# micropilot/myosuite-mjx

Hardware: AMD Instinct MI355X
Metric: env-steps/s (whole node) myoHandPoseRandom-v0 batch 4096 (higher is better)
Workload: dtype f32

## Files before the change

__graft_entry__.py:

```python
import os
import subprocess
import sys

ROOT = os.path.dirname(os.path.abspath(__file__))
sys.path.insert(0, ROOT)


def build() -> None:
    from myosuite_mjx_amd import capi
    capi.build_library(force=True, verbose=True)
    capi.build_diagnostic("poison", verbose=True)
    subprocess.check_call(["make", "-C", os.path.join(ROOT, "oracle"), "-s"])
    if os.path.isdir("/root/reference/myosuite") and os.environ.get("MYO_RECOMPILE_MODELS") == "1":
        subprocess.check_call([sys.executable, os.path.join(ROOT, "tools", "compile_models.py")])
    import myosuite_mjx_amd
    import ctypes
    lib = ctypes.CDLL(capi.LIB_PATH)
    for sym in ("myo_model_load", "myo_batch_create", "myo_step", "myo_obs", "myo_reset"):
        getattr(lib, sym)
    print("build ok:", capi.LIB_PATH)


def smoke() -> None:
    import numpy as np
    from myosuite_mjx_amd import capi, model as M
    from oracle.oracle import Oracle
# ... 32 lines not shown
```

include/myo_hip.h:

```cpp
#ifndef MYO_HIP_H
#define MYO_HIP_H
#include <stddef.h>
#include <stdint.h>
#ifdef __cplusplus
extern "C" {
#endif

typedef struct myo_model myo_model;
typedef struct myo_batch myo_batch;

enum { MYO_OK = 0, MYO_E_ARG = -1, MYO_E_BLOB = -2, MYO_E_HIP = -3, MYO_E_UNSUPPORTED = -4, MYO_E_NOMEM = -5 };

typedef struct myo_dims {
  int nq, nv, nu, na, nbody, ntendon, nsite, nlink, obs_dim, env_lds_bytes, lanes_per_env, ncon_max;
  float timestep;
} myo_dims;

typedef enum myo_field {
  MYO_F_QPOS = 0,
  MYO_F_QVEL,
  MYO_F_ACT,
  MYO_F_CTRL,
  MYO_F_WARMSTART,
  MYO_F_TIME,
// ... 19 lines not shown
  MYO_F_BODYMASS_RANGE,
  MYO_F_COUNT
} myo_field;

enum {
  MYO_F_BODYPOS = MYO_F_COUNT,
  MYO_F_BODYPOS_RANGE,
};

enum { MYO_FLAG_BAD_STATE = 1, MYO_FLAG_BAD_QACC = 2, MYO_FLAG_CONTACT_OVERFLOW = 4, MYO_FLAG_CAND_OVERFLOW = 8,
       MYO_FLAG_SCHED_TIMEOUT = 16  };

enum {
  MYO_F_BODYQUAT = MYO_F_BODYPOS_RANGE + 1,
  MYO_F_BODYQUAT_RANGE,
};

enum {
  MYO_ACTMAP_NONE = 0,
  MYO_ACTMAP_MUSCLE_SIGMOID = 1,
  MYO_ACTMAP_SIGMOID_FATIGUE = 2,
  MYO_ACTMAP_SIGMOID_REAFFERENTATION = 3,
  MYO_ACTMAP_CTRLRANGE = 4
};

typedef enum myo_task { MYO_TASK_NONE = 0, MYO_TASK_POSE = 1, MYO_TASK_REACH = 2, MYO_TASK_WALK = 3,
                        MYO_TASK_STAND = 5,
                        MYO_TASK_TRACK = 6,
                        MYO_TASK_KEYTURN = 7,
                        MYO_TASK_PEN = 8,
// ... 120 lines not shown
```

myosuite_mjx_amd/capi.py:

```python
from __future__ import annotations

import ctypes as C
import os
import subprocess

import numpy as np

_HERE = os.path.dirname(os.path.abspath(__file__))
LIB_PATH = os.environ.get("MYO_HIP_LIB") or os.path.join(_HERE, "libmyo_hip.so")
SRC_PATH = os.path.join(_HERE, "csrc", "myo_hip.hip")

(F_QPOS, F_QVEL, F_ACT, F_CTRL, F_WARMSTART, F_TIME, F_TARGET, F_OBS, F_REWARD, F_DONE, F_SOLVED, F_FLAGS, F_DIAG,
 F_QACC, F_TENLEN, F_ACTFORCE, F_SITEXPOS, F_ELAPSED, F_ACTION, F_FATIGUE, F_HFIELD, F_GEOMSIZE, F_LINKX, F_METRICS,
 F_BODYMASS, F_BODYMASS_RANGE, F_BODYPOS, F_BODYPOS_RANGE) = range(28)
F_BODYQUAT, F_BODYQUAT_RANGE = 28, 29
INT_FIELDS = (F_FLAGS, F_DIAG, F_ELAPSED)
BENCH_OBS, BENCH_FRESH_ACTIONS, BENCH_AUTORESET = 1, 2, 4
ACTMAP_NONE, ACTMAP_MUSCLE_SIGMOID, ACTMAP_SIGMOID_FATIGUE, ACTMAP_SIGMOID_REAFFERENTATION, ACTMAP_CTRLRANGE = 0, 1, 2, 3, 4
TASK_NONE, TASK_POSE, TASK_REACH = 0, 1, 2
TASK_HOLD = 4
TASK_STAND = 5
TASK_TRACK = 6
TASK_KEYTURN = 7
TASK_PEN = 8
TASK_BAODING = 9
TASK_DIE = 10
FLAG_BAD_STATE, FLAG_BAD_QACC, FLAG_CONTACT_OVERFLOW, FLAG_CAND_OVERFLOW = 1, 2, 4, 8


class Dims(C.Structure):
    _fields_ = [(n, C.c_int) for n in ("nq", "nv", "nu", "na", "nbody", "ntendon", "nsite", "nlink", "obs_dim",
# ... 50 lines not shown
def build_library(force=False, verbose=False):
    csrc = os.path.dirname(SRC_PATH)
    newest = max(os.path.getmtime(os.path.join(csrc, f)) for f in os.listdir(csrc) if f.endswith((".hip", ".h")))
    newest = max(newest, os.path.getmtime(os.path.join(os.path.dirname(os.path.dirname(csrc)), "include", "myo_hip.h")))
    if not force and os.path.exists(LIB_PATH) and os.path.getmtime(LIB_PATH) >= newest:
        return LIB_PATH
    hipcc = os.environ.get("HIPCC", "/opt/rocm/bin/hipcc")
    cmd = [hipcc, *HIPCC_FLAGS, "-shared", "-fPIC", "-o", LIB_PATH, SRC_PATH]
    if verbose:
        print(" ".join(cmd))
    subprocess.check_call(cmd)
    return LIB_PATH


def build_diagnostic(variant, force=False, verbose=False):
    flag = {"poison": "-DMYO_POISON=1", "stamps": "-DMYO_STAMPS=1"}[variant]
    out = os.path.join(os.path.dirname(LIB_PATH), f"libmyo_hip_{variant}.so")
    csrc = os.path.dirname(SRC_PATH)
    newest = max(os.path.getmtime(os.path.join(csrc, f)) for f in os.listdir(csrc) if f.endswith((".hip", ".h")))
    if not force and os.path.exists(out) and os.path.getmtime(out) >= newest:
        return out
    hipcc = os.environ.get("HIPCC", "/opt/rocm/bin/hipcc")
    cmd = [hipcc, *HIPCC_FLAGS, flag, "-shared", "-fPIC", "-o", out, SRC_PATH]
    if verbose:
        print(" ".join(cmd))
    subprocess.check_call(cmd)
    return out


_lib = None

# ... 314 lines not shown
```

myosuite_mjx_amd/csrc/myo_common.h:

```cpp
#ifndef MYO_COMMON_H
#define MYO_COMMON_H

#include <hip/hip_runtime.h>

#include <algorithm>
#include <utility>
#include <cmath>
#include <cstdint>
#include <cstdio>
#include <cstdlib>
#include <cstring>
#include <mutex>
#include <string>
#include <vector>

#include "../../include/myo_hip.h"

#define MINVALF 1e-15f
#define MAXVALF 1e10f
#define MINIMPF 0.0001f
#define MAXIMPF 0.9999f
#define NCON 32
#define NCAND 128
#ifndef LS_FLOOR
// ... 72 lines not shown
  float obj_p[3], obj_R[9], wrist_p[3];
  float lift_z, obj_err_scale, base_err_scale, lift_bonus_mag, qpos_w, qpos_err_scale, qvel_w, qvel_err_scale;
  float obj_fail2, base_fail2, qpos_fail;
  float w_pose, w_object, w_bonus, w_penalty;
  float* ref;
  int ref_pitch;
  float* metrics;
  uint64_t seed;
};

struct DevBatch {
  int B;
  float *qpos, *qvel, *act, *ctrl, *warm, *time, *target, *obs, *reward, *done, *solved, *qacc, *tenlen, *actforce, *sitexpos;
  int *flags, *diag, *elapsed, *episode;
  int* mprw;
  float* fatigue;
  float fat_dt;
  int reaf_epl, reaf_eip;
  float* hfield;
  float* gsize;
  int gsize_cg;
  float* bmass;
  float* bmass_range;
  float* linkc;
  int nbody;
  float* bpos;
  float* bpos_range;
  int bpos_link;
  float* ovf;
  int* ovf_cand;
// ... 163 lines not shown
```

myosuite_mjx_amd/csrc/myo_hip.hip:

```cpp
#include "myo_common.h"
#include "myo_physics.h"
#include "myo_task_track.h"
#include "myo_kernel_lanes.h"
#include "myo_kernel_wave.h"
#include "myo_kernels_aux.h"
#include "myo_host.h"
#include "myo_task_keyturn.h"
#include "myo_task_pen.h"
#include "myo_task_baoding.h"
#include "myo_task_die.h"
#include "myo_task_myodm.h"
#include "myo_host_model.h"

extern "C" {

const char* myo_last_error(void) { return g_err.c_str(); }
int myo_version(void) { return 1; }

int myo_model_load(const void* blobv, size_t nbytes, int device, myo_model** out) {
  if (!blobv || !out || nbytes < 16) return fail(MYO_E_ARG, "myo_model_load: bad arguments");
  const Blob B{(const uint8_t*)blobv};
  uint32_t ver;
  memcpy(&ver, B.p + 4, 4);
  if (memcmp(B.p, "MYOB", 4) || ver != 3) return fail(MYO_E_BLOB, "myo_model_load: not a MYOB v3 blob");
// ... 44 lines not shown
  DevBatch& d = b->db;
  d.B = B;
  int nv = m->dm.nv, nu = m->dm.nu, nq = m->nq, rc;
  b->ntarget_alloc = nv > 24 ? nv : 24;
  b->obs_alloc = 3 * nv + 4 * nu + 64;
#define BA(ptr, n) if ((rc = balloc(b, (void**)&ptr, (size_t)(n) * 4))) { myo_batch_free(b); return rc; }
  BA(d.qpos, (size_t)B * nq) BA(d.qvel, (size_t)B * nv) BA(d.act, (size_t)B * nu) BA(d.ctrl, (size_t)B * nu) BA(d.warm, (size_t)B * nv)
  BA(d.time, B) BA(d.target, (size_t)B * b->ntarget_alloc) BA(d.obs, (size_t)B * b->obs_alloc) BA(d.reward, B) BA(d.done, B)
  BA(d.solved, B) BA(d.qacc, (size_t)B * nv) BA(d.tenlen, (size_t)B * nu) BA(d.actforce, (size_t)B * nu) BA(d.sitexpos, (size_t)B * 24)
  BA(d.flags, B) BA(d.diag, (size_t)B * 8) BA(d.elapsed, B) BA(d.episode, B) BA(d.mprw, (size_t)B * 64)
  BA(b->d_tlo, b->ntarget_alloc) BA(b->d_thi, b->ntarget_alloc) BA(b->d_init, nq) BA(b->d_jlo, nv) BA(b->d_jhi, nv) BA(b->d_rnd, 4 * (size_t)nq)
  BA(b->d_action, (size_t)B * nu)
  BA(d.fatigue, (size_t)B * 3 * nu)
  d.hfield = nullptr; d.gsize = nullptr; d.gsize_cg = -1;
  d.ovf = nullptr; d.ovf_cand = nullptr; d.ovf_row = 0; d.ovf_rows = 0; d.linkx = nullptr; d.track = nullptr; d.env_offset = 0;
  if (m->trk) { BA(d.linkx, (size_t)B * 12 * m->dm.nl) }
  if (m->wave_ok) {
    const int kc = m->wave_cfg == 0 ? 8 : 20, nj = m->trk ? 4 : 3;
    d.ovf_row = 8 + nj * kc + (kc + 3) / 4 + (m->trk ? TRK_STATE : 0);
    d.ovf_rows = m->trk ? NCX2 : NCX;
    BA(d.ovf, (size_t)B * d.ovf_rows * d.ovf_row) BA(d.ovf_cand, (size_t)B * NCANDX)
  }
  if (m->dw.hf.on) { BA(d.hfield, (size_t)B * m->dw.hf.nrow * m->dw.hf.ncol) }
  BA(b->d_initv, nv) BA(b->d_init2, nq) BA(b->d_initv2, nv) BA(b->d_fatvec, nu)
  { void* pw = nullptr; if ((rc = balloc(b, &pw, sizeof(DevWalk)))) { myo_batch_free(b); return rc; } b->d_walk = (DevWalk*)pw; }
  BA(b->d_stamps, (size_t)B * 12 * 3 * 2)
  BA(b->d_order, B)
  b->sched_stride = (B + 7) / 8 + 1;
  BA(b->d_sched, 32 + B + 64)
#undef BA
// ... 316 lines not shown
    case MYO_F_ACT: *p = d.act; *pitch = *width = nu; break;
    case MYO_F_CTRL: *p = d.ctrl; *pitch = *width = nu; break;
    case MYO_F_WARMSTART: *p = d.warm; *pitch = *width = nv; break;
    case MYO_F_TIME: *p = d.time; *pitch = *width = 1; break;
    case MYO_F_TARGET: *p = d.target; *pitch = *width = b->task.ntarget > 0 ? b->task.ntarget : 1; break;
    case MYO_F_OBS: *p = d.obs; *pitch = *width = b->task.obs_dim > 0 ? b->task.obs_dim : 1; break;
    case MYO_F_REWARD: *p = d.reward; *pitch = *width = 1; break;
    case MYO_F_DONE: *p = d.done; *pitch = *width = 1; break;
    case MYO_F_SOLVED: *p = d.solved; *pitch = *width = 1; break;
    case MYO_F_FLAGS: *p = d.flags; *pitch = *width = 1; break;
    case MYO_F_DIAG: *p = d.diag; *pitch = *width = 8; break;
    case MYO_F_QACC: *p = d.qacc; *pitch = *width = nv; break;
    case MYO_F_TENLEN: *p = d.tenlen; *pitch = *width = nu; break;
    case MYO_F_ACTFORCE: *p = d.actforce; *pitch = *width = nu; break;
    case MYO_F_ELAPSED: *p = d.elapsed; *pitch = *width = 1; break;
    case MYO_F_LINKX:
      if (!d.linkx) return fail(MYO_E_ARG, "MYO_F_LINKX: this model's kernel does not export link frames");
      *p = d.linkx; *pitch = *width = (size_t)12 * b->model->dm.nl; break;
    case MYO_F_ACTION: *p = b->d_action; *pitch = *width = nu; break;
    case MYO_F_FATIGUE: *p = d.fatigue; *pitch = *width = 3 * nu; break;
    case MYO_F_GEOMSIZE:
      if (!d.gsize) return fail(MYO_E_ARG, "MYO_F_GEOMSIZE: no geom override set (myo_batch_set_geom_override)");
      *p = d.gsize; *pitch = *width = 4; break;
    case MYO_F_HFIELD:
      if (!d.hfield) return fail(MYO_E_ARG, "MYO_F_HFIELD: the model has no colliding height field");
      *p = d.hfield; *pitch = *width = b->model->dw.hf.nrow * b->model->dw.hf.ncol; break;
    case MYO_F_METRICS:
      if (!b->d_metrics) return fail(MYO_E_ARG, "MYO_F_METRICS: the track task is not configured (myo_batch_configure_track)");
      *p = b->d_metrics; *pitch = *width = 4; break;
    case MYO_F_SITEXPOS: *p = d.sitexpos; *pitch = *width = b->task.ntip > 0 ? 3 * b->task.ntip : 1; break;
// ... 556 lines not shown
```

myosuite_mjx_amd/csrc/myo_host_model.h:

```cpp
#ifndef MYO_HOST_MODEL_H
#define MYO_HOST_MODEL_H

struct BlobRec { char name[32]; uint32_t dtype, ndim, shape[4]; uint64_t nbytes, offset; };

struct Blob {
  const uint8_t* p;
  mutable int rc = MYO_OK;
  const BlobRec* find(const char* name) const {
    uint32_t n;
    memcpy(&n, p + 8, 4);
    for (uint32_t i = 0; i < n; i++) {
      const BlobRec* r = (const BlobRec*)(p + 16 + (size_t)i * sizeof(BlobRec));
      if (!strncmp(r->name, name, 32)) return r;
    }
    return nullptr;
  }
  bool has(const char* name) const { return find(name) != nullptr; }
  template <class Src, class Dst> std::vector<Dst> read(const char* name, uint32_t dtype) const {
    const BlobRec* r = find(name);
    if (!r || r->dtype != dtype) {
      if (!rc) rc = fail(MYO_E_BLOB, std::string("model blob lacks ") + (dtype ? "i32" : "f64") + " array " + name);
      return {};
    }
    const Src* s = (const Src*)(p + r->offset);
// ... 156 lines not shown
  if (bb > 0 && jt.size() == jb.size() && (jt.back() == 2 || jt.back() == 3)
      && bb < (int)bp.size() && bb < (int)bl.size() && bp[bb] == 0) {
    const int l = bl[bb];
    bool head = l >= 0 && l < (int)lpar.size() && lpar[l] < 0;
    for (int k = 1; head && k < bb; k++) if (bl[k] == l) head = false;
    if (head) m->bp_link = l;
  }
  return MYO_OK;
}

static float bits_f(int v) { float f; memcpy(&f, &v, 4); return f; }

struct PackedModel {
  std::vector<float> seg_rec, cg_rec, pair_rec;
  std::vector<int> dl_pk, pair_dl_pk, kin_pk, link_desc, link_adof, dof_anc;
};

static int pack_segments(const myo_model* m, const Blob& B, PackedModel* P) {
  const DevModel& d = m->dm;
  const std::vector<int> seg = B.ints("hip_seg"), seg_order = B.ints("hip_seg_order"), seg_tendon = B.ints("hip_seg_tendon"), wg_link = B.ints("hip_wg_link"), dl = B.ints("hip_dl");
  const std::vector<float> seg_div = B.floats("hip_seg_div"), site_lpos = B.floats("hip_site_lpos"), wg_lpos = B.floats("hip_wg_lpos"), wg_lmat = B.floats("hip_wg_lmat"), wg_radius = B.floats("hip_wg_radius");
  if (B.rc) return B.rc;
  const std::vector<int>&site_link = m->site_link, &dof_type = m->dof_type;
  std::vector<int> dlp(std::max<size_t>(dl.size() / 3, 1), 0);
  for (size_t i = 0; i < dl.size() / 3; i++) {
    const int dd = dl[3 * i], sg = dl[3 * i + 1], slot = dl[3 * i + 2];
    if (dd < 0 || dd > 127 || slot < 0 || slot > 255 || sg < -32768 || sg > 32767) return fail(MYO_E_UNSUPPORTED, "moment-arm list entry does not fit the packed word");
    dlp[i] = dd | ((dof_type[dd] == 3 ? 1 : 0) << 7) | (slot << 8) | (int)((unsigned)sg << 16);
  }
  std::vector<int>& dl4 = P->dl_pk;
// ... 35 lines not shown
  for (int g = 0; g < d.ncg; g++) {
    float* R = &P->cg_rec[(size_t)g * 16];
    R[0] = bits_f(cg_link[g]); for (int c = 0; c < 3; c++) R[1 + c] = cg_lpos[3 * (size_t)g + c];
    for (int c = 0; c < 9; c++) R[4 + c] = cg_lmat[9 * (size_t)g + c];
    R[13] = bits_f(cg_type[g]); R[14] = cg_rb[g];
  }
  for (int q = 0; q < d.npair; q++) {
    const int* I = &pair_i[6 * (size_t)q];
    const float* F = &pair_f[12 * (size_t)q];
    if (I[0] > 255 || I[1] > 255 || I[3] > 255 || I[4] > 15 || I[5] > 15) return fail(MYO_E_UNSUPPORTED, "collision pair does not fit the packed pair record");
    float* R = &P->pair_rec[(size_t)q * 16];
    R[0] = bits_f(I[0] | (I[1] << 8) | (I[4] << 16) | (I[5] << 20) | (I[3] << 24)); R[1] = F[0]; R[2] = F[1]; R[3] = bits_f(I[2]);
    for (int c = 0; c < 3; c++) { R[4 + c] = cg_size[3 * (size_t)I[0] + c]; R[8 + c] = cg_size[3 * (size_t)I[1] + c]; }
    R[7] = cg_rb[I[0]]; R[11] = cg_rb[I[1]];
    R[12] = bits_f(cg_type[I[0]] | (cg_type[I[1]] << 8));
  }
  if (d.npair > 2048 || pair_dl.size() / 2 >= (1u << 16) || d.maxkc > 31) return fail(MYO_E_UNSUPPORTED, "more than 2048 collision pairs, 65535 contact dof-list entries or 31 dofs per contact");
  P->pair_dl_pk.assign(std::max<size_t>(pair_dl.size() / 2, 1), 0);
  for (size_t i = 0; i < pair_dl.size() / 2; i++) {
    const int dd = pair_dl[2 * i], sg = pair_dl[2 * i + 1];
    if (dd < 0 || dd > 127 || sg < -(1 << 22) || sg > (1 << 22)) return fail(MYO_E_UNSUPPORTED, "contact dof-list entry does not fit the packed word");
    P->pair_dl_pk[i] = dd | ((dof_type[dd] == 3 ? 1 : 0) << 7) | (int)((unsigned)sg << 8);
  }
  return MYO_OK;
}

static int pack_tree(myo_model* m, const Blob& B, const std::vector<int>& dpar, PackedModel* P) {
  const DevModel& d = m->dm;
  DevModelW& w = m->dw;
  const std::vector<int> kadr = B.ints("hip_kin_adr"), kvec = B.ints("hip_kin_vec"), chadr = B.ints("hip_link_chain_adr"), chain = B.ints("hip_link_chain");
// ... 109 lines not shown
}

static int load_model(myo_model* m, const Blob& B) {
  DevModel& d = m->dm;
  DevModelW& w = m->dw;
  int rc;
  if ((rc = load_header(m, B)) || (rc = load_tables(m, B))) return rc;
  if (m->trk && (rc = load_body_tables(m, B))) return rc;
  const std::vector<int> pair_i = B.ints("hip_pair_i"), dpar = B.ints("dof_parentid");
  for (int p = 0; p < d.npair; p++) {
    if ((pair_i[6 * p + 4] == 6 || pair_i[6 * p + 4] == 7) && !m->trk) return fail(MYO_E_UNSUPPORTED, "plane - cylinder pairs need a model of the TrackEnv class");
    if (pair_i[6 * p + 4] == 8 && !m->trk) return fail(MYO_E_UNSUPPORTED, "plane - sphere pairs need a model of the TrackEnv class");
  }
  PackedModel P;
  if ((rc = pack_segments(m, B, &P)) || (rc = pack_collision(m, B, &P)) || (rc = pack_tree(m, B, dpar, &P))) return rc;
  if ((rc = upload(m, P.seg_rec, &w.seg_rec)) || (rc = upload(m, P.dl_pk, &w.dl_pk)) || (rc = upload(m, P.cg_rec, &w.cg_rec)) ||
      (rc = upload(m, P.pair_rec, &w.pair_rec)) || (rc = upload(m, P.pair_dl_pk, &w.pair_dl_pk)) || (rc = upload(m, P.kin_pk, &w.kin_pk)) ||
      (rc = upload(m, P.link_desc, &w.link_desc)) || (rc = upload(m, P.link_adof, &w.link_adof)) || (rc = upload(m, P.dof_anc, &w.dof_anc))) return rc;
  if (B.has("integrator")) { const std::vector<int> ig = B.ints("integrator"); if (B.rc) return B.rc; m->rk4 = !ig.empty() && ig[0] == 1; }
  if ((rc = classify(m, pair_i, dpar))) return rc;
  void* p1 = nullptr; void* p2 = nullptr;
  if (hipMalloc(&p1, sizeof(DevModel)) == hipSuccess) m->dev_allocs.push_back(p1);
  if (hipMalloc(&p2, sizeof(DevModelW)) == hipSuccess) m->dev_allocs.push_back(p2);
  if (!p1 || !p2) return fail(MYO_E_NOMEM, "hipMalloc model structs");
  m->d_dm = (DevModel*)p1; m->d_dw = (DevModelW*)p2;
  if (hipMemcpy(p1, &d, sizeof(DevModel), hipMemcpyHostToDevice) != hipSuccess || hipMemcpy(p2, &w, sizeof(DevModelW), hipMemcpyHostToDevice) != hipSuccess) return fail(MYO_E_HIP, "upload model structs");
  m->dims.na = d.na_obs;
  m->dims.env_lds_bytes = m->wave_ok ? m->env_lds_bytes_w : m->env_lds_bytes;
  m->dims.ncon_max = m->wave_ok ? (m->wave_cfg >= 1 ? 32 : NCONW) : NCON;
  if (m->wave_ok && !m->body_link.empty() && (rc = load_body_mass_tables(m, B))) return rc;
// ... 5 lines not shown
```

myosuite_mjx_amd/csrc/myo_kernel_wave.h:

```cpp
#ifndef MYO_KERNEL_WAVE_H
#define MYO_KERNEL_WAVE_H

#define NCONW 32
#define MPRW 14
static_assert(4 * MPRW <= 63, "the scheduler carries the table in a 64-word row (word 63 = entry count)");
struct LayW {
  int qpos, qvel, act, ctrl, lpos, lmat, axis, anchor, xv, qfc, sq, mprw, X;
  int tJ, tlen, tforce;
  int cdof, cinert, crb, cvel, cacc, cfrc;
  int gpos, gax, cand, cdist, cpos, cnrm, cpair, cJ, cdofs;
  int Mp;
  int tJp;
  int total;
};
__host__ __device__ constexpr LayW layout_w(int nq, int nv, int nu, int nl, int ngt, int maxnnz, int ncg, bool has_tl, int nvt, int kc, int nc, int nj) {
  LayW Y{};
  int o = 0;
  Y.qpos = o; o += nq; Y.qvel = o; o += nv; Y.act = o; o += nu; Y.ctrl = o; o += nu;
  Y.lpos = o; o += 3 * nl; Y.lmat = o; o += 9 * nl; Y.axis = o; o += 3 * nv; Y.anchor = o; o += 3 * nv;
  Y.xv = o; o += nvt; Y.qfc = o; o += nvt; Y.sq = o; o += nvt * (nvt + 1); Y.mprw = o; o += 4 * MPRW;
  Y.tJp = 0;
  if (has_tl) { Y.tJp = o; o += ngt * maxnnz + 2 * ngt; }
  Y.X = o;
  Y.tJ = o; o += ngt * maxnnz; Y.tlen = o; o += ngt; Y.tforce = o; o += nu;
  const int endT = o;
  o = Y.X;
  Y.cdof = o; o += 6 * nv; Y.cinert = o; o += 10 * nl; Y.crb = o; o += 10 * nl; Y.cvel = o; o += 6 * nl; Y.cacc = o; o += 6 * nl; Y.cfrc = o; o += 6 * nl;
  const int endD = o;
  o = Y.X;
  Y.Mp = o;
  Y.gpos = o; o += 3 * ncg; Y.gax = o; o += 3 * ncg;
  Y.cand = o; o += NCAND;
  if (o - Y.Mp < (nvt * (nvt + 1)) / 2) o = Y.Mp + (nvt * (nvt + 1)) / 2;
  Y.cdist = o; o += nc; Y.cpos = o; o += 3 * nc; Y.cnrm = o; o += 3 * nc; Y.cpair = o; o += nc;
  Y.cJ = o; o += nc * nj * kc; Y.cdofs = o; o += nc * ((kc + 3) / 4);
// ... 18 lines not shown
  gpi kin_base, kin_adr, kin_vec;
  gpf eq_f;
  gpf mesh_rec, mesh_startrec, mesh_aabb;
  gpf fl, mesh_vert;
  gpf4 seg_rec;
  gpi dl_pk;
  gpf4 cg_rec;
  gpf4 pair_rec;
  gpi pair_dl_pk;
  gpi kin_pk;
  int kin_nround;
  gpi link_desc;
  gpi link_adof;
  gpi dof_anc;
  unsigned int free_rot[2], free_j3[2];
};
#define SEGR 9
#ifndef MPR_TOL
#define MPR_TOL 1e-8f
#endif

__device__ __forceinline__ float rdlane(float v, int l) { return __int_as_float(__builtin_amdgcn_readlane(__float_as_int(v), l)); }
__device__ __forceinline__ int rdlanei(int v, int l) { return __builtin_amdgcn_readlane(v, l); }
__device__ __forceinline__ float uniformf(float v) { return __int_as_float(__builtin_amdgcn_readfirstlane(__float_as_int(v))); }
template <int CTRL> __device__ __forceinline__ float dpp_add(float v) {
  return v + __int_as_float(__builtin_amdgcn_update_dpp(0, __float_as_int(v), CTRL, 0xf, 0xf, true));
}
__device__ __forceinline__ float wave_sum(float v) {
  v = dpp_add<0xB1>(v);
  v = dpp_add<0x4E>(v);
// ... 267 lines not shown
template <> struct Sizes<3> { static constexpr int nq = 35, nv = 34, nu = 80, nl = 13, nlevel = 6, maxnnz = 11, nseg = 100, ncg = 33, npair = 76; };
template <int SPEC> static bool sizes_match(int nq, int nv, int nu, int nl, int nlevel, int maxnnz, int ngt, int nseg, int ncg, int npair) {
  typedef Sizes<SPEC> Z;
  return nq == Z::nq && nv == Z::nv && nu == Z::nu && nl == Z::nl && nlevel == Z::nlevel && maxnnz == Z::maxnnz && ngt == Z::nu && nseg == Z::nseg &&
         ncg == Z::ncg && npair == Z::npair;
}

template <int SPEC, int NVT, int KC, int NC, int NJ> struct LayC {
  typedef Sizes<SPEC> Z;
  static constexpr LayW L = layout_w(Z::nq, Z::nv, Z::nu, Z::nl, Z::nu, Z::maxnnz, Z::ncg, false, NVT, KC, NC, NJ);
  static constexpr int qpos = L.qpos, qvel = L.qvel, act = L.act, ctrl = L.ctrl, lpos = L.lpos, lmat = L.lmat, axis = L.axis, anchor = L.anchor, xv = L.xv,
                       qfc = L.qfc, sq = L.sq, mprw = L.mprw, X = L.X, tJ = L.tJ, tlen = L.tlen, tforce = L.tforce, cdof = L.cdof, cinert = L.cinert, crb = L.crb,
                       cvel = L.cvel, cacc = L.cacc, cfrc = L.cfrc, gpos = L.gpos, gax = L.gax, cand = L.cand, cdist = L.cdist, cpos = L.cpos, cnrm = L.cnrm,
                       cpair = L.cpair, cJ = L.cJ, cdofs = L.cdofs, Mp = L.Mp, tJp = L.tJp, total = L.total;
};
template <int SPEC, int NVT, int KC, int NC, int NJ> static bool layout_match(const LayW& a) {
  const LayW b = layout_w(Sizes<SPEC>::nq, Sizes<SPEC>::nv, Sizes<SPEC>::nu, Sizes<SPEC>::nl, Sizes<SPEC>::nu, Sizes<SPEC>::maxnnz, Sizes<SPEC>::ncg, false, NVT, KC, NC, NJ);
  return memcmp(&a, &b, sizeof(LayW)) == 0;
}

template <int NVT, int KC, int NC, int NTR, int WPE, bool SCHED, int SPEC, bool HF = false, bool TRK = false, bool RK4 = false>
__global__ void __launch_bounds__(64, WPE) step_kernel_w(const DevModel* __restrict__ Mp, const DevModelW* __restrict__ Wp, DevBatch Bt,
                                                        const float* __restrict__ action, int actmap, int nsub, long long* stamps,
                                                        const int* __restrict__ order, const DevWalk* __restrict__ wk, int kflags, SchedDev S) {
  extern __shared__ __align__(16) float E[];
  const DevModel& M = *Mp;
  const DevModelW& W = *Wp;
  const LayC<SPEC, NVT, KC, NC, (TRK ? 4 : 3)> Yc{};
  const auto& Y = [&]() -> const auto& { if constexpr (SPEC != 0) return Yc; else return W.lay; }();
#define lane_id wave_lane()
// ... 2 lines not shown
  if (!SCHED) {
    switch (oe >> 28) {
      case 3: __builtin_amdgcn_s_setprio(3); break;
      case 2: __builtin_amdgcn_s_setprio(2); break;
      case 1: __builtin_amdgcn_s_setprio(1); break;
      default: break;
    }
  }
  typedef Sizes<SPEC> Z;
  const int nv = SPEC ? Z::nv : M.nv, nu = SPEC ? Z::nu : M.nu, nq = SPEC ? Z::nq : W.nq;
  const int nl_ = SPEC ? Z::nl : M.nl, nlevel_ = SPEC ? Z::nlevel : M.nlevel, maxnnz_ = SPEC ? Z::maxnnz : M.maxnnz, ngt_ = SPEC ? Z::nu : M.ngt,
            nseg_ = SPEC ? Z::nseg : M.nseg, ncg_ = SPEC ? Z::ncg : M.ncg, npair_ = SPEC ? Z::npair : M.npair;
  constexpr int CDW = (KC + 3) / 4;
  constexpr int NJ = TRK ? 4 : 3;
  constexpr int NR = TRK ? 6 : 4;
  constexpr bool FULL = NVT > 24;
  const bool has_free = FULL && W.has_free;
  const int neq = FULL ? W.neq : 0;
  const bool has_tl = (SPEC != 0 || TRK) ? false : (W.has_tl != 0);
  const bool walk = FULL && wk != nullptr;
  if (!SCHED && FULL && (kflags & KF_RESET_ONLY) && Bt.elapsed[env] != 0) return;
#if MYO_STAMPS
  long long st_acc[12] = {0, 0, 0, 0, 0, 0, 0, 0, 0, 0, 0, 0};
  long long st_t0 = clock64();
  long long st_sub[12] = {0, 0, 0, 0, 0, 0, 0, 0, 0, 0, 0, 0}, st_s0 = 0;
  long long st_x[12] = {0, 0, 0, 0, 0, 0, 0, 0, 0, 0, 0, 0};
#define SUB0() do { st_s0 = clock64(); } while (0)
#define SUB(k) do { long long t1_ = clock64(); st_sub[k] += t1_ - st_s0; st_s0 = t1_; } while (0)
#define SUBX(k) do { long long t1_ = clock64(); st_x[k] += t1_ - st_s0; st_s0 = t1_; } while (0)
#define CNTX(k) do { st_x[k]++; } while (0)
// ... 80 lines not shown
      if (L.g1 == Bt.gsize_cg) { L.s1[0] = G[0]; L.s1[1] = G[1]; L.s1[2] = G[2]; L.rb1 = G[3]; }
      if (L.g2 == Bt.gsize_cg) { L.s2[0] = G[0]; L.s2[1] = G[1]; L.s2[2] = G[2]; L.rb2 = G[3]; }
    }
    return L;
  };
  auto pair_load = [&](int p) -> PairL { return pair_decode(pair_raw(p)); };
  constexpr int NCXK = TRK ? (128 - NC) : ((64 - NC) < NCX ? (64 - NC) : NCX);
  float* const ovf_env = Bt.ovf ? Bt.ovf + (size_t)env * Bt.ovf_rows * Bt.ovf_row : nullptr;
  const int ovf_row = Bt.ovf_row;
  const int nct = ovf_env ? NC + NCXK : NC;
  constexpr int RND = (NC * NJ * KC >= 768) ? 64 : 32;
  static_assert(RND * 12 <= NC * NJ * KC, "MPR scratch must fit the contact-jacobian area");
  int* const ovf_cand = (!HF && Bt.ovf_cand) ? Bt.ovf_cand + (size_t)env * NCANDX : nullptr;
  bool alive = true;
  int n_mprw = 0;
  if (SCHED && s0 > 0) {
    const int* Wt = Bt.mprw + (size_t)env * 64;
    n_mprw = __builtin_amdgcn_readfirstlane(ldstatei<SCHED>(Wt + 63));
    if (lane_id < 4 * n_mprw) ((int*)(E + Y.mprw))[lane_id] = ldstatei<SCHED>(Wt + lane_id);
  }
  SYNC();
  static_assert(!(RK4 && SCHED), "the substep scheduler hands out Euler substeps");
  for (int step = s0; step < s1; step++) {
    const bool op = walk && step == nsub;
    float rk_v0 = 0.f, rk_q0 = 0.f, rk_sv = 0.f, rk_sa = 0.f, rk_t0 = 0.f, rk_quat[4] = {1.f, 0.f, 0.f, 0.f}, rk_a0[NTR], rk_sd[NTR];
#pragma unroll
    for (int rr = 0; rr < NTR; rr++) { rk_a0[rr] = 0.f; rk_sd[rr] = 0.f; }
    int rk_stage = 0;
  rk_next_stage:
    asm volatile("" ::: "memory");
// ... 569 lines not shown
        if (HF) {
          unsigned long long hb = __ballot(nh > 0);
          int myat = 0;
          while (hb) {
            const int L = __ffsll((long long)hb) - 1;
            hb &= hb - 1ull;
            if (lane == L) myat = ncand;
            ncand += rdlanei(nh, L);
          }
          if (nh > 0) hf_walk(W.hf, Bt.hfield + (size_t)env * W.hf.nrow * W.hf.ncol, hr0, hr1, hc0, hc1, hzcut, p, cand, myat, NCAND);
        }
      }
      { const int candcap = ovf_cand ? NCAND + NCANDX : NCAND; if (ncand > candcap) { flags |= MYO_FLAG_CAND_OVERFLOW; ncand = candcap; } }
      f_cand += ncand;
      int n_mprw_new = 0;
      SYNC();
      STAMP(6);
      MeshTab MT;
      if constexpr (TRK) { MT.vert = W.mesh_vert; MT.rec = (gpf4)W.mesh_rec; MT.srec = (gpf4)W.mesh_startrec; }
      for (int base = 0; base < ncand; base += RND) {
        int ci = (RND == 64 || lane < RND) ? base + lane : ncand;
        int nsup = -8;
        bool mpr_hit = false;
        float mpr_n[3] = {0.f, 0.f, 0.f};
        bool hit = false, hit2 = false;
        float dist = 0, dist2 = 0, cpos[3] = {0, 0, 0}, cpos2[3] = {0, 0, 0}, nrm[3] = {1, 0, 0};
        int p = -1, cword = 0;
        if (ci < ncand) {
          const int cw = (ci < NCAND) ? cand[ci] : ovf_cand[ci - NCAND];
          p = HF ? (cw & 1023) : cw;
// ... 197 lines not shown
            else pen = mpr_penetration(o1, o2, MPR_TOL, 60, &depth, dir, pos, &nsup, have_nw ? nw : nullptr);
            if (pen) {
              dist = margin - depth;
              normalize3(dir);
              mpr_hit = !prism; mpr_n[0] = dir[0]; mpr_n[1] = dir[1]; mpr_n[2] = dir[2];
              float dw[3], pw[3];
              matvec(dw, R1, dir);
              matvec(pw, R1, pos);
#pragma unroll
              for (int k = 0; k < 3; k++) { cpos[k] = pw[k] + x1[k] + (prism ? cen[k] : 0.f); nrm[k] = dw[k]; }
              hit = true;
            }
                      } else {
            const float zero3[3] = {0.f, 0.f, 0.f};
            nsup = 0;
            float R1[9];
            geom_world_mat(W, Y, E, g1, R1, brp);
            CObj o1, o2;
            {
              float R2[9], rel[3] = {x2[0] - x1[0], x2[1] - x1[1], x2[2] - x1[2]};
              geom_world_mat(W, Y, E, g2, R2, brp);
#pragma unroll
              for (int i = 0; i < 3; i++)
#pragma unroll
                for (int j = 0; j < 3; j++) o2.mat[3 * i + j] = R1[i] * R2[j] + R1[3 + i] * R2[3 + j] + R1[6 + i] * R2[6 + j];
              matTvec(o2.pos, R1, rel);
            }
#pragma unroll
            for (int k = 0; k < 9; k++) o1.mat[k] = (k == 0 || k == 4 || k == 8) ? 1.f : 0.f;
#pragma unroll
            for (int k = 0; k < 3; k++) o1.pos[k] = 0.f;
            if constexpr (TRK) {
              cobj_shape_poly(o1, Q.t1, sz1);
              cobj_shape_poly(o2, Q.t2, sz2);
            }
            else { cobj_shape(o1, Q.t1, sz1); cobj_shape(o2, Q.t2, sz2); }
            o1.margin = o2.margin = 0.5f * margin;
            float depth, dir[3], pos[3], nw[3] = {0.f, 0.f, 0.f};
            bool have_nw = false;
            for (int i = 0; i < n_mprw; i++) {
              if (((const int*)(E + Y.mprw))[4 * i] == p) { nw[0] = E[Y.mprw + 4 * i + 1]; nw[1] = E[Y.mprw + 4 * i + 2]; nw[2] = E[Y.mprw + 4 * i + 3]; have_nw = true; }
            }
            if (mpr_penetration_wl<TRK ? 2 : 0>(o1, o2, MPR_TOL, 60, &depth, dir, pos, &nsup, have_nw ? nw : nullptr, E + Y.cJ + 12 * lane, MT)) {
              dist = margin - depth;
              normalize3(dir);
              mpr_hit = true; mpr_n[0] = dir[0]; mpr_n[1] = dir[1]; mpr_n[2] = dir[2];
              float dw[3], pw[3], R1b[9];
              geom_world_mat(W, Y, E, g1, R1b, brp);
              matvec(dw, R1b, dir);
              matvec(pw, R1b, pos);
#pragma unroll
              for (int k = 0; k < 3; k++) { cpos[k] = pw[k] + x1[k]; nrm[k] = dw[k]; }
              hit = true;
            }
                      }
          }
          if (hit && !(dist < margin - Q.gap)) hit = false;
          if (hit2 && !(dist2 < margin - Q.gap)) hit2 = false;
        }
        {
          int w = nsup + 8;
          w = max(w, __builtin_amdgcn_update_dpp(0, w, 0xB1, 0xf, 0xf, true));
          w = max(w, __builtin_amdgcn_update_dpp(0, w, 0x4E, 0xf, 0xf, true));
          w = max(w, __builtin_amdgcn_update_dpp(0, w, 0x141, 0xf, 0xf, true));
          w = max(w, __builtin_amdgcn_update_dpp(0, w, 0x140, 0xf, 0xf, true));
          f_mpr += max(max(rdlanei(w, 0), rdlanei(w, 16)), max(rdlanei(w, 32), rdlanei(w, 48)));
        }
        {
          SYNC();
          unsigned long long wb = __ballot(mpr_hit);
          int wpos = n_mprw_new + __popcll(wb & ((1ull << lane) - 1ull));
          if (mpr_hit && wpos < MPRW) {
            ((int*)(E + Y.mprw))[4 * wpos] = p;
            E[Y.mprw + 4 * wpos + 1] = mpr_n[0]; E[Y.mprw + 4 * wpos + 2] = mpr_n[1]; E[Y.mprw + 4 * wpos + 3] = mpr_n[2];
          }
          n_mprw_new = min(n_mprw_new + (int)__popcll(wb), MPRW);
        }
        unsigned long long bal = __ballot(hit);
        int pos = ncon + __popcll(bal & ((1ull << lane) - 1ull));
        if (hit && pos < NC) {
          E[Y.cdist + pos] = dist;
#pragma unroll
          for (int k = 0; k < 3; k++) { E[Y.cpos + 3 * pos + k] = cpos[k]; E[Y.cnrm + 3 * pos + k] = nrm[k]; }
// ... 15 lines not shown
            for (int k = 0; k < 3; k++) { E[Y.cpos + 3 * pos + k] = cpos2[k]; E[Y.cnrm + 3 * pos + k] = nrm[k]; }
            ((int*)(E + Y.cpair))[pos] = cword;
          } else if (hit2 && pos < nct) {
            float* g = ovf_env + (pos - NC) * ovf_row;
            g[0] = dist2;
#pragma unroll
            for (int k = 0; k < 3; k++) { g[1 + k] = cpos2[k]; g[4 + k] = nrm[k]; }
            ((int*)g)[7] = cword;
          }
          ncon += __popcll(bal);
        }
      }
      if (ncon > nct) { flags |= MYO_FLAG_CONTACT_OVERFLOW; ncon = nct; }
      n_mprw = n_mprw_new;
      SYNC();
    } else n_mprw = 0;
    STAMP(4);
    const float warm_r = lane < nv ? ldstate<SCHED>(warm_row + lane) : 0.f;
    float lsign = 0.f, laref = 0.f, lD = 0.f;
    if (lane < nv && !M.disable_limit) {
      const float* J = M.jl + 12 * lane;
      if (J[0] != 0) {
        float q = E[Y.qpos + W.dof_qposadr[lane]], margin = J[3];
        float dlo = q - J[1], dhi = J[2] - q, dist = 0;
        if (dlo < margin && dlo <= dhi) { lsign = 1; dist = dlo; }
        else if (dhi < margin) { lsign = -1; dist = dhi; }
        if (lsign != 0) {
          float imp = impedance(J + 6, dist, margin), K, B;
          float R = fmaxf(MINVALF, (1 - imp) / imp * J[11]);
          kbi(J[4], J[5], J[7], M.timestep, &K, &B);
          laref = -B * (lsign * E[Y.qvel + lane]) - K * imp * (dist - margin);
// ... 881 lines not shown
  }
  if (lane_id < nq) Bt.qpos[(size_t)env * nq + lane_id] = E[Y.qpos + lane_id];
  if (lane_id < nv) {
    Bt.qvel[(size_t)env * nv + lane_id] = E[Y.qvel + lane_id];
    Bt.qacc[(size_t)env * nv + lane_id] = warm_row[lane_id];
  }
  for (int i = lane_id; i < nu; i += 64) {
    Bt.act[(size_t)env * nu + i] = E[Y.act + i];
    Bt.ctrl[(size_t)env * nu + i] = E[Y.ctrl + i];
  }
  if (SCHED && s1 < nsubtot) {
    int* Wt = Bt.mprw + (size_t)env * 64;
    if (lane_id < 4 * n_mprw) Wt[lane_id] = ((const int*)(E + Y.mprw))[lane_id];
    if (lane_id == 63) Wt[63] = n_mprw;
  }
  if (lane_id == 0) {
    Bt.time[env] = time;
    if (s1 == nsubtot) Bt.elapsed[env] = track_reset ? 0 : Bt.elapsed[env] + 1;
    if (SCHED) { if (flags) atomicOr(&Bt.flags[env], flags); } else Bt.flags[env] |= flags;
    Bt.diag[(size_t)env * 8 + 0] = d_nefc; Bt.diag[(size_t)env * 8 + 1] = d_ncon; Bt.diag[(size_t)env * 8 + 2] = d_iter;
    d_cost = FULL ? 1909 + ((7436 * f_cand - 28892 * f_ncon + 1362 * f_mpr + 25014 * f_iter + 2046 * f_itcon - 1413 * f_ls + 13292 * d_nefc + 343707 * d_ncon) >> 10)
                  : 2236 + ((-141 * f_cand - 3413 * f_ncon + 2188 * f_mpr + 8971 * f_iter - 107 * f_itcon - 122 * f_ls - 518 * d_nefc + 74475 * d_ncon) >> 10);
    d_cost = max(d_cost, 1);
    Bt.diag[(size_t)env * 8 + 3] = d_cost;
    Bt.diag[(size_t)env * 8 + 4] = f_cand | (f_ncon << 16); Bt.diag[(size_t)env * 8 + 5] = f_mpr;
    Bt.diag[(size_t)env * 8 + 6] = f_itcon | (f_iter << 16); Bt.diag[(size_t)env * 8 + 7] = f_ls | (f_fact << 16);
  }
  last_cost = d_cost;
  STAMP(9);
  if (!SCHED) break;
// ... 19 lines not shown
```

Baseline: 4.474 million.

## Move MPR warm-start table from LDS to per-env global memory for small models

For models whose kernel config is not the full-size/non-tracking one (e.g. MyoHand), the MPR warm-start normals are stored in a per-environment global array indexed by collision pair, stamped with a substep tick. This replaces the LDS table with its linear search and SYNC, shrinking the LDS slice per env, which may raise occupancy. In exchange it adds global loads and stores per collision pair and a tick counter written each substep. A capped diagnostic variant is also built.

```diff
diff --git a/__graft_entry__.py b/__graft_entry__.py
--- a/__graft_entry__.py
+++ b/__graft_entry__.py
@@ -10,6 +10,7 @@
     from myosuite_mjx_amd import capi
     capi.build_library(force=True, verbose=True)
     capi.build_diagnostic("poison", verbose=True)
+    capi.build_diagnostic("mprcap", verbose=True)
     subprocess.check_call(["make", "-C", os.path.join(ROOT, "oracle"), "-s"])
     if os.path.isdir("/root/reference/myosuite") and os.environ.get("MYO_RECOMPILE_MODELS") == "1":
         subprocess.check_call([sys.executable, os.path.join(ROOT, "tools", "compile_models.py")])
diff --git a/include/myo_hip.h b/include/myo_hip.h
--- a/include/myo_hip.h
+++ b/include/myo_hip.h
@@ -57,6 +57,10 @@
 enum {
   MYO_F_BODYQUAT = MYO_F_BODYPOS_RANGE + 1,
   MYO_F_BODYQUAT_RANGE,
+};
+
+enum {
+  MYO_F_MPRWARM = MYO_F_BODYQUAT_RANGE + 1
 };
 
 enum {
diff --git a/myosuite_mjx_amd/capi.py b/myosuite_mjx_amd/capi.py
--- a/myosuite_mjx_amd/capi.py
+++ b/myosuite_mjx_amd/capi.py
@@ -14,7 +14,8 @@
  F_QACC, F_TENLEN, F_ACTFORCE, F_SITEXPOS, F_ELAPSED, F_ACTION, F_FATIGUE, F_HFIELD, F_GEOMSIZE, F_LINKX, F_METRICS,
  F_BODYMASS, F_BODYMASS_RANGE, F_BODYPOS, F_BODYPOS_RANGE) = range(28)
 F_BODYQUAT, F_BODYQUAT_RANGE = 28, 29
-INT_FIELDS = (F_FLAGS, F_DIAG, F_ELAPSED)
+F_MPRWARM = 30
+INT_FIELDS = (F_FLAGS, F_DIAG, F_ELAPSED, F_MPRWARM)
 BENCH_OBS, BENCH_FRESH_ACTIONS, BENCH_AUTORESET = 1, 2, 4
 ACTMAP_NONE, ACTMAP_MUSCLE_SIGMOID, ACTMAP_SIGMOID_FATIGUE, ACTMAP_SIGMOID_REAFFERENTATION, ACTMAP_CTRLRANGE = 0, 1, 2, 3, 4
 TASK_NONE, TASK_POSE, TASK_REACH = 0, 1, 2
@@ -95,7 +96,7 @@
 
 
 def build_diagnostic(variant, force=False, verbose=False):
-    flag = {"poison": "-DMYO_POISON=1", "stamps": "-DMYO_STAMPS=1"}[variant]
+    flag = {"poison": "-DMYO_POISON=1", "stamps": "-DMYO_STAMPS=1", "mprcap": "-DMYO_MPR_WARM_CAP=14"}[variant]
     out = os.path.join(os.path.dirname(LIB_PATH), f"libmyo_hip_{variant}.so")
     csrc = os.path.dirname(SRC_PATH)
     newest = max(os.path.getmtime(os.path.join(csrc, f)) for f in os.listdir(csrc) if f.endswith((".hip", ".h")))
diff --git a/myosuite_mjx_amd/csrc/myo_common.h b/myosuite_mjx_amd/csrc/myo_common.h
--- a/myosuite_mjx_amd/csrc/myo_common.h
+++ b/myosuite_mjx_amd/csrc/myo_common.h
@@ -110,6 +110,8 @@
   float *qpos, *qvel, *act, *ctrl, *warm, *time, *target, *obs, *reward, *done, *solved, *qacc, *tenlen, *actforce, *sitexpos;
   int *flags, *diag, *elapsed, *episode;
   int* mprw;
+  float* mprn;
+  int mprn_pitch;
   float* fatigue;
   float fat_dt;
   int reaf_epl, reaf_eip;
diff --git a/myosuite_mjx_amd/csrc/myo_hip.hip b/myosuite_mjx_amd/csrc/myo_hip.hip
--- a/myosuite_mjx_amd/csrc/myo_hip.hip
+++ b/myosuite_mjx_amd/csrc/myo_hip.hip
@@ -82,6 +82,11 @@
   BA(d.fatigue, (size_t)B * 3 * nu)
   d.hfield = nullptr; d.gsize = nullptr; d.gsize_cg = -1;
   d.ovf = nullptr; d.ovf_cand = nullptr; d.ovf_row = 0; d.ovf_rows = 0; d.linkx = nullptr; d.track = nullptr; d.env_offset = 0;
+  d.mprn = nullptr; d.mprn_pitch = 0;
+  if (m->wave_ok && m->wave_cfg != 1) {
+    d.mprn_pitch = m->dw.n_mpr_pairs + 1;
+    BA(d.mprn, (size_t)B * d.mprn_pitch * 4)
+  }
   if (m->trk) { BA(d.linkx, (size_t)B * 12 * m->dm.nl) }
   if (m->wave_ok) {
     const int kc = m->wave_cfg == 0 ? 8 : 20, nj = m->trk ? 4 : 3;
@@ -428,6 +433,9 @@
     case MYO_F_TENLEN: *p = d.tenlen; *pitch = *width = nu; break;
     case MYO_F_ACTFORCE: *p = d.actforce; *pitch = *width = nu; break;
     case MYO_F_ELAPSED: *p = d.elapsed; *pitch = *width = 1; break;
+    case MYO_F_MPRWARM:
+      if (!d.mprn) return fail(MYO_E_ARG, "MYO_F_MPRWARM: this model's kernel keeps its MPR warm-start table in LDS");
+      *p = d.mprn; *pitch = *width = (size_t)4 * d.mprn_pitch; break;
     case MYO_F_LINKX:
       if (!d.linkx) return fail(MYO_E_ARG, "MYO_F_LINKX: this model's kernel does not export link frames");
       *p = d.linkx; *pitch = *width = (size_t)12 * b->model->dm.nl; break;
diff --git a/myosuite_mjx_amd/csrc/myo_host_model.h b/myosuite_mjx_amd/csrc/myo_host_model.h
--- a/myosuite_mjx_amd/csrc/myo_host_model.h
+++ b/myosuite_mjx_amd/csrc/myo_host_model.h
@@ -194,6 +194,7 @@
 struct PackedModel {
   std::vector<float> seg_rec, cg_rec, pair_rec;
   std::vector<int> dl_pk, pair_dl_pk, kin_pk, link_desc, link_adof, dof_anc;
+  int n_mpr_pairs = 0;
 };
 
 static int pack_segments(const myo_model* m, const Blob& B, PackedModel* P) {
@@ -259,6 +260,7 @@
     for (int c = 0; c < 3; c++) { R[4 + c] = cg_size[3 * (size_t)I[0] + c]; R[8 + c] = cg_size[3 * (size_t)I[1] + c]; }
     R[7] = cg_rb[I[0]]; R[11] = cg_rb[I[1]];
     R[12] = bits_f(cg_type[I[0]] | (cg_type[I[1]] << 8));
+    if (I[4] == 0 || I[4] == 4) P->n_mpr_pairs = q + 1;
   }
   if (d.npair > 2048 || pair_dl.size() / 2 >= (1u << 16) || d.maxkc > 31) return fail(MYO_E_UNSUPPORTED, "more than 2048 collision pairs, 65535 contact dof-list entries or 31 dofs per contact");
   P->pair_dl_pk.assign(std::max<size_t>(pair_dl.size() / 2, 1), 0);
@@ -398,6 +400,7 @@
   }
   PackedModel P;
   if ((rc = pack_segments(m, B, &P)) || (rc = pack_collision(m, B, &P)) || (rc = pack_tree(m, B, dpar, &P))) return rc;
+  w.n_mpr_pairs = P.n_mpr_pairs;
   if ((rc = upload(m, P.seg_rec, &w.seg_rec)) || (rc = upload(m, P.dl_pk, &w.dl_pk)) || (rc = upload(m, P.cg_rec, &w.cg_rec)) ||
       (rc = upload(m, P.pair_rec, &w.pair_rec)) || (rc = upload(m, P.pair_dl_pk, &w.pair_dl_pk)) || (rc = upload(m, P.kin_pk, &w.kin_pk)) ||
       (rc = upload(m, P.link_desc, &w.link_desc)) || (rc = upload(m, P.link_adof, &w.link_adof)) || (rc = upload(m, P.dof_anc, &w.dof_anc))) return rc;
diff --git a/myosuite_mjx_amd/csrc/myo_kernel_wave.h b/myosuite_mjx_amd/csrc/myo_kernel_wave.h
--- a/myosuite_mjx_amd/csrc/myo_kernel_wave.h
+++ b/myosuite_mjx_amd/csrc/myo_kernel_wave.h
@@ -3,6 +3,11 @@
 
 #define NCONW 32
 #define MPRW 14
+__host__ __device__ constexpr bool mprw_in_lds(int nvt, int nj) { return nvt > 24 && nj == 3; }
+#ifndef MYO_MPR_WARM_CAP
+#define MYO_MPR_WARM_CAP 0
+#endif
+static_assert(MYO_MPR_WARM_CAP >= 0 && MYO_MPR_WARM_CAP <= 15, "the capped build keeps a hit's rank in four bits of its stamp");
 static_assert(4 * MPRW <= 63, "the scheduler carries the table in a 64-word row (word 63 = entry count)");
 struct LayW {
   int qpos, qvel, act, ctrl, lpos, lmat, axis, anchor, xv, qfc, sq, mprw, X;
@@ -18,7 +23,7 @@
   int o = 0;
   Y.qpos = o; o += nq; Y.qvel = o; o += nv; Y.act = o; o += nu; Y.ctrl = o; o += nu;
   Y.lpos = o; o += 3 * nl; Y.lmat = o; o += 9 * nl; Y.axis = o; o += 3 * nv; Y.anchor = o; o += 3 * nv;
-  Y.xv = o; o += nvt; Y.qfc = o; o += nvt; Y.sq = o; o += nvt * (nvt + 1); Y.mprw = o; o += 4 * MPRW;
+  Y.xv = o; o += nvt; Y.qfc = o; o += nvt; Y.sq = o; o += nvt * (nvt + 1); Y.mprw = o; if (mprw_in_lds(nvt, nj)) o += 4 * MPRW;
   Y.tJp = 0;
   if (has_tl) { Y.tJp = o; o += ngt * maxnnz + 2 * ngt; }
   Y.X = o;
@@ -67,6 +72,7 @@
   gpi link_adof;
   gpi dof_anc;
   unsigned int free_rot[2], free_j3[2];
+  int n_mpr_pairs;
 };
 #define SEGR 9
 #ifndef MPR_TOL
@@ -364,6 +370,9 @@
                        cvel = L.cvel, cacc = L.cacc, cfrc = L.cfrc, gpos = L.gpos, gax = L.gax, cand = L.cand, cdist = L.cdist, cpos = L.cpos, cnrm = L.cnrm,
                        cpair = L.cpair, cJ = L.cJ, cdofs = L.cdofs, Mp = L.Mp, tJp = L.tJp, total = L.total;
 };
+static_assert(LayC<1, 24, 8, 32, 3>::total == 2502, "MyoHand LDS slice");
+static_assert(LayC<2, 36, 20, 32, 3>::total == 5051, "MyoLeg LDS slice");
+static_assert(LayC<3, 36, 20, 32, 3>::total == 5051, "terrain LDS slice");
 template <int SPEC, int NVT, int KC, int NC, int NJ> static bool layout_match(const LayW& a) {
   const LayW b = layout_w(Sizes<SPEC>::nq, Sizes<SPEC>::nv, Sizes<SPEC>::nu, Sizes<SPEC>::nl, Sizes<SPEC>::nu, Sizes<SPEC>::maxnnz, Sizes<SPEC>::ncg, false, NVT, KC, NC, NJ);
   return memcmp(&a, &b, sizeof(LayW)) == 0;
@@ -396,6 +405,8 @@
   constexpr int CDW = (KC + 3) / 4;
   constexpr int NJ = TRK ? 4 : 3;
   constexpr int NR = TRK ? 6 : 4;
+  constexpr bool MPRG = !mprw_in_lds(NVT, NJ);
+  static_assert(!(SCHED && MPRG), "the scheduler carries the LDS table between its tasks");
   constexpr bool FULL = NVT > 24;
   const bool has_free = FULL && W.has_free;
   const int neq = FULL ? W.neq : 0;
@@ -506,6 +517,13 @@
   int* const ovf_cand = (!HF && Bt.ovf_cand) ? Bt.ovf_cand + (size_t)env * NCANDX : nullptr;
   bool alive = true;
   int n_mprw = 0;
+  auto mprn_row = [&]() -> float4* { return (float4*)Bt.mprn + (size_t)env * Bt.mprn_pitch; };
+  auto mpr_tick = [&]() -> int {
+    volatile int* const c = (volatile int*)mprn_row();
+    const int t = __builtin_amdgcn_readfirstlane(*c) + 1;
+    if (lane_id == 0) *c = t;
+    return t;
+  };
   if (SCHED && s0 > 0) {
     const int* Wt = Bt.mprw + (size_t)env * 64;
     n_mprw = __builtin_amdgcn_readfirstlane(ldstatei<SCHED>(Wt + 63));
@@ -1105,6 +1123,8 @@
       { const int candcap = ovf_cand ? NCAND + NCANDX : NCAND; if (ncand > candcap) { flags |= MYO_FLAG_CAND_OVERFLOW; ncand = candcap; } }
       f_cand += ncand;
       int n_mprw_new = 0;
+      int mpr_t = 0;
+      if constexpr (MPRG) mpr_t = mpr_tick();
       SYNC();
       STAMP(6);
       MeshTab MT;
@@ -1332,6 +1352,8 @@
                       } else {
             const float zero3[3] = {0.f, 0.f, 0.f};
             nsup = 0;
+            float4 wrec = make_float4(0.f, 0.f, 0.f, 0.f);
+            if constexpr (MPRG) { if (p + 1 < Bt.mprn_pitch) wrec = mprn_row()[1 + p]; }
             float R1[9];
             geom_world_mat(W, Y, E, g1, R1, brp);
             CObj o1, o2;
@@ -1356,8 +1378,18 @@
             o1.margin = o2.margin = 0.5f * margin;
             float depth, dir[3], pos[3], nw[3] = {0.f, 0.f, 0.f};
             bool have_nw = false;
+            if constexpr (MPRG) {
+              const unsigned int sw = (unsigned int)__float_as_int(wrec.x);
+#if MYO_MPR_WARM_CAP
+              have_nw = sw != 0u && (sw >> 4) == (unsigned int)(mpr_t - 1) && (int)(sw & 15u) >= n_mprw_new;
+#else
+              have_nw = sw != 0u && sw == (unsigned int)(mpr_t - 1);
+#endif
+              nw[0] = wrec.y; nw[1] = wrec.z; nw[2] = wrec.w;
+            } else {
             for (int i = 0; i < n_mprw; i++) {
               if (((const int*)(E + Y.mprw))[4 * i] == p) { nw[0] = E[Y.mprw + 4 * i + 1]; nw[1] = E[Y.mprw + 4 * i + 2]; nw[2] = E[Y.mprw + 4 * i + 3]; have_nw = true; }
+            }
             }
             if (mpr_penetration_wl<TRK ? 2 : 0>(o1, o2, MPR_TOL, 60, &depth, dir, pos, &nsup, have_nw ? nw : nullptr, E + Y.cJ + 12 * lane, MT)) {
               dist = margin - depth;
@@ -1384,7 +1416,16 @@
           w = max(w, __builtin_amdgcn_update_dpp(0, w, 0x140, 0xf, 0xf, true));
           f_mpr += max(max(rdlanei(w, 0), rdlanei(w, 16)), max(rdlanei(w, 32), rdlanei(w, 48)));
         }
-        {
+        if constexpr (MPRG) {
+#if MYO_MPR_WARM_CAP
+          const unsigned long long wb = __ballot(mpr_hit);
+          const int wpos = n_mprw_new + __popcll(wb & ((1ull << lane) - 1ull));
+          if (mpr_hit && wpos < MYO_MPR_WARM_CAP && p + 1 < Bt.mprn_pitch) *(int4*)(mprn_row() + 1 + p) = make_int4((int)(((unsigned int)mpr_t << 4) | (unsigned int)wpos), __float_as_int(mpr_n[0]), __float_as_int(mpr_n[1]), __float_as_int(mpr_n[2]));
+          n_mprw_new = min(n_mprw_new + (int)__popcll(wb), MYO_MPR_WARM_CAP);
+#else
+          if (mpr_hit && p + 1 < Bt.mprn_pitch) mprn_row()[1 + p] = make_float4(__int_as_float(mpr_t), mpr_n[0], mpr_n[1], mpr_n[2]);
+#endif
+        } else {
           SYNC();
           unsigned long long wb = __ballot(mpr_hit);
           int wpos = n_mprw_new + __popcll(wb & ((1ull << lane) - 1ull));
@@ -1430,7 +1471,7 @@
       if (ncon > nct) { flags |= MYO_FLAG_CONTACT_OVERFLOW; ncon = nct; }
       n_mprw = n_mprw_new;
       SYNC();
-    } else n_mprw = 0;
+    } else { n_mprw = 0; if constexpr (MPRG) mpr_tick(); }
     STAMP(4);
     const float warm_r = lane < nv ? ldstate<SCHED>(warm_row + lane) : 0.f;
     float lsign = 0.f, laref = 0.f, lD = 0.f;
@@ -2342,6 +2383,7 @@
     if (lane_id < 4 * n_mprw) Wt[lane_id] = ((const int*)(E + Y.mprw))[lane_id];
     if (lane_id == 63) Wt[63] = n_mprw;
   }
+  if constexpr (MPRG) mpr_tick();
   if (lane_id == 0) {
     Bt.time[env] = time;
     if (s1 == nsubtot) Bt.elapsed[env] = track_reset ? 0 : Bt.elapsed[env] + 1;
```

Result: no change. 4.451 million (-0.5%).
